# LimpBunion22/VIT-FPGA

Measured on AMD Instinct MI355X. Metric: images/sec ViT-B/16 224x224, batch 512 per GPU, higher is better.
Workload: dtype bf16; 1 GPU; vit_base 224x224x3 inference, 512 images per GPU resident in HBM, random-init weights (seed 0); global_batch=512, per_gpu_batch=512

## Files before the change

### vit-fpga_amd/csrc/kernels_attn.hip

```cpp
#include <type_traits>

#include "attn_common.h"

namespace vh {

template <typename T, typename TO = T>
__global__ void __launch_bounds__(1024, 4)
attention_kernel(const typename T::elem* __restrict__ qkv, typename TO::elem* __restrict__ out,
                 int tokens, int heads, int slabs, int ntiles) {
    using elem = typename T::elem;
    using vec8 = typename T::vec8;
    using vec4 = typename T::vec4;
    extern __shared__ __attribute__((aligned(16))) char smem[];
    const int kv_bytes = ntiles * 4096;

    const int lane = threadIdx.x & 63;
    const int wave = __builtin_amdgcn_readfirstlane(threadIdx.x >> 6);
    const int nw = blockDim.x >> 6;
    const int l31 = lane & 31, hl = lane >> 5;
    const int D = heads * 64;
    const int64_t ld = 3 * (int64_t)D;

    const int lr = lane >> 3, pc = lane & 7;
    const int ngroups = ntiles * 4;

    const int koff = l31 * 128;
    const int kswz = (l31 >> 1) & 7;
    const int g4 = lane >> 4, i16 = lane & 15, tq = i16 >> 2, tp = i16 & 3;
    const int vrow0 = 4 * (g4 >> 1) + tq;
    const int vcolb = (16 * (g4 & 1) + 4 * tp) * 2;

    const int item = blockIdx.x;
    const int bh = item / slabs, slab = item - bh * slabs;
    const int b = bh / heads, h = bh - b * heads;
    const int q0 = (slab * nw + wave) * 32;

    auto issue_kv = [&]() {
        const elem* base = qkv + (int64_t)b * tokens * ld + h * 64;
        for (int g = wave; g < ngroups; g += nw) {
            const int row = g * 8 + lr;
            const int rsrc = row < tokens ? row : tokens - 1;
            const elem* src = base + rsrc * ld;
            const int ck = pc ^ ((row >> 1) & 7);
            const int cv = pc ^ (((row >> 1) & 1) << 2);
            __builtin_amdgcn_global_load_lds((const void __attribute__((address_space(1)))*)(src + D + ck * 8),
                                             (void __attribute__((address_space(3)))*)(smem + g * 1024), 16, 0, 0);
            __builtin_amdgcn_global_load_lds((const void __attribute__((address_space(1)))*)(src + 2 * D + cv * 8),
                                             (void __attribute__((address_space(3)))*)(smem + kv_bytes + g * 1024), 16, 0, 0);
        }
    };
    vec8 qf[4];
    auto load_q = [&]() {
        int qrow = q0 + l31;
        qrow = qrow < tokens ? qrow : tokens - 1;
        const elem* qp = qkv + ((int64_t)b * tokens + qrow) * ld + h * 64 + 8 * hl;
#pragma unroll
        for (int ks = 0; ks < 4; ++ks) qf[ks] = *(const vec8*)(qp + 16 * ks);
    };
    issue_kv();
    load_q();

    asm volatile("s_waitcnt vmcnt(0)" ::: "memory");
    __syncthreads();
    const char* Ks = smem;
    const char* Vs = Ks + kv_bytes;

    if (q0 < tokens) {
        f32x16 o0, o1;
#pragma unroll
        for (int r = 0; r < 16; ++r) { o0[r] = 0.f; o1[r] = 0.f; }
        float m2 = -INFINITY;
        float lsum = 0.f;

        const char* kbase = Ks + koff;
        int kofs[4];
#pragma unroll
        for (int ks = 0; ks < 4; ++ks) kofs[ks] = ((2 * ks + hl) ^ kswz) << 4;
        const int vx = ((vrow0 >> 1) & 1) << 6;
        const char* vb0 = Vs + vrow0 * 128 + (vcolb ^ vx);
        const char* vb1 = Vs + vrow0 * 128 + ((vcolb + 64) ^ vx);

        auto qk = [&](int kt) {
            f32x16 s;
#pragma unroll
            for (int r = 0; r < 16; ++r) s[r] = 0.f;
            const char* kp = kbase + kt * 4096;
#pragma unroll
            for (int ks = 0; ks < 4; ++ks) s = T::mfma32(*(const vec8*)(kp + kofs[ks]), qf[ks], s);
            return s;
        };
        struct VFrag { vec8 f[2][2]; };
        auto load_v = [&](int kt) {
            VFrag v;
            const char* v0 = vb0 + kt * 4096;
            const char* v1 = vb1 + kt * 4096;
#pragma unroll
            for (int ks = 0; ks < 2; ++ks) {
                const vec4 a0 = T::tr_read(v0 + ks * 2048), c0 = T::tr_read(v0 + ks * 2048 + 1024);
                const vec4 a1 = T::tr_read(v1 + ks * 2048), c1 = T::tr_read(v1 + ks * 2048 + 1024);
#pragma unroll
                for (int j = 0; j < 4; ++j) { v.f[ks][0][j] = a0[j]; v.f[ks][0][4 + j] = c0[j]; v.f[ks][1][j] = a1[j]; v.f[ks][1][4 + j] = c1[j]; }
            }
            return v;
        };
        auto softmax_pv = [&](int kt, f32x16 s, const VFrag& vfr, auto masked) {
            if constexpr (decltype(masked)::value) {
#pragma unroll
                for (int r = 0; r < 16; ++r) {
                    const int key = kt * 32 + (r & 3) + 8 * (r >> 2) + 4 * hl;
                    if (key >= tokens) s[r] = -INFINITY;
                }
            }
            float mx = s[0];
#pragma unroll
            for (int r = 1; r < 16; ++r) mx = fmaxf(mx, s[r]);
            mx = cross_half_max(mx);
            const float mnew = fmaxf(m2, mx);
            if (__builtin_amdgcn_ballot_w64(mnew != m2)) {
                const float alpha = __builtin_amdgcn_exp2f(m2 - mnew);
                lsum *= alpha;
#pragma unroll
                for (int r = 0; r < 16; ++r) { o0[r] *= alpha; o1[r] *= alpha; }
                m2 = mnew;
            }
            float psum = 0.f;
#pragma unroll
            for (int r = 0; r < 16; ++r) {
                s[r] = __builtin_amdgcn_exp2f(s[r] - mnew);
                psum += s[r];
            }
            lsum += psum;
#pragma unroll
            for (int ks = 0; ks < 2; ++ks) {
                vec8 pf;
#pragma unroll
                for (int j = 0; j < 8; ++j) pf[j] = (elem)s[8 * ks + j];
                o0 = T::mfma32(vfr.f[ks][0], pf, o0);
                o1 = T::mfma32(vfr.f[ks][1], pf, o1);
            }
        };
        f32x16 s_cur = qk(0);
        for (int kt = 0; kt + 1 < ntiles; ++kt) {
            const VFrag vfr = load_v(kt);
            const f32x16 s_nxt = qk(kt + 1);
            softmax_pv(kt, s_cur, vfr, std::false_type{});
            s_cur = s_nxt;
        }
        {
            const VFrag vfr = load_v(ntiles - 1);
            softmax_pv(ntiles - 1, s_cur, vfr, std::true_type{});
        }

        const float ltot = cross_half_sum(lsum);
        const float inv = 1.0f / ltot;
        const int q = q0 + l31;
        if (q < tokens) {
            typename TO::elem* op = out + ((int64_t)b * tokens + q) * D + h * 64 + 4 * hl;
#pragma unroll
            for (int rg = 0; rg < 4; ++rg) {
                *(typename TO::vec4*)(op + 8 * rg) = pack4<TO>(o0[4 * rg] * inv, o0[4 * rg + 1] * inv, o0[4 * rg + 2] * inv, o0[4 * rg + 3] * inv);
                *(typename TO::vec4*)(op + 32 + 8 * rg) = pack4<TO>(o1[4 * rg] * inv, o1[4 * rg + 1] * inv, o1[4 * rg + 2] * inv, o1[4 * rg + 3] * inv);
            }
        }
    }
}

#ifndef VH_ATTN_ABL
#define VH_ATTN_ABL 0
#endif
__device__ __forceinline__ void ring_dma16(const void* base, uint32_t lane_off, uint32_t lds_addr) {
    asm_lds_dma16(base, lane_off, lds_addr);
}
#ifdef VH_DIAG_STAMPS
__device__ unsigned long long g_attn_diag[1024 * 16 * 16];
__device__ __forceinline__ unsigned long long attn_rt() {
    unsigned long long t;
    asm volatile("s_memrealtime %0\n\ts_waitcnt lgkmcnt(0)" : "=s"(t)::"memory");
    return t;
}
__device__ __forceinline__ unsigned long long attn_ct() {
    unsigned long long t;
    asm volatile("s_memtime %0\n\ts_waitcnt lgkmcnt(0)" : "=s"(t)::"memory");
    return t;
}
#define VH_ATT_T(i) do { __builtin_amdgcn_sched_barrier(0); const unsigned long long n_ = attn_ct(); ph_[i] += n_ - last_; last_ = n_; __builtin_amdgcn_sched_barrier(0); } while (0)
#else
#define VH_ATT_T(i) do { } while (0)
#endif
__device__ __forceinline__ void ring_wait_vm(int n) { wait_vm<40>(n); }
__device__ __forceinline__ void ring_wait_dma() {
    asm volatile("s_waitcnt vmcnt(0)" ::: "memory");
}

template <typename T, typename TO = T, bool QS = false, bool OTILE = false, bool IHM = false>
__global__ void __launch_bounds__(1024, 4)
attention_ring_kernel(const typename T::elem* __restrict__ qkv, typename TO::elem* __restrict__ out,
                      int tokens, int heads, int slabs, int ntiles, int nitems, unsigned int* __restrict__ ticket,
                      unsigned int heads_rcp, int64_t hm_rows) {
    using elem = typename T::elem;
    using vec8 = typename T::vec8;
    using vec4 = typename T::vec4;
    extern __shared__ __attribute__((aligned(16))) char smem[];
    const int G = (tokens + 7) >> 3, G2 = (G + 1) & ~1;
    const int kv_bytes = QS ? G * 1024 : ntiles * 4096;
    const int q_off = kv_bytes + (QS ? G2 * 1024 : kv_bytes);
    const uint32_t lds0 = (uint32_t)(uintptr_t)smem;

    const int lane = threadIdx.x & 63;
    const int wave = __builtin_amdgcn_readfirstlane(threadIdx.x >> 6);
    const int nw = blockDim.x >> 6;
    const int l31 = lane & 31, hl = lane >> 5;
    const int D = heads * 64;
    const int64_t ld = IHM ? 64 : 3 * (int64_t)D;
    const uint32_t koff2 = IHM ? (uint32_t)(hm_rows * D * 2) : (uint32_t)(D * 2);
    auto head_base = [&](int b, int h) {
        if constexpr (IHM) return qkv + ((int64_t)h * hm_rows + (int64_t)b * tokens) * 64;
        else return qkv + (int64_t)b * tokens * ld + h * 64;
    };

    auto kv_base = [&](int item) {
        if (QS) {
            const int b = (heads == 1 ? item : (int)__umulhi((unsigned)item, heads_rcp)), h = item - b * heads;
            return head_base(b, h);
        }
        const int bh = item / slabs;
        const int b = bh / heads, h = bh - b * heads;
        return head_base(b, h);
    };
    auto issue_tile = [&](const elem* base, int t) {
        int ln = lane;
        asm volatile("" : "+v"(ln));
        const int lr_ = ln >> 3, pc_ = ln & 7;
        const int g = 4 * t + wave;
        const int gk = QS && g >= G ? G - 1 : g, gv = QS && g >= G2 ? G2 - 1 : g;
        const int rowk = gk * 8 + lr_, rowv = gv * 8 + lr_;
        const int rk = rowk < tokens ? rowk : tokens - 1;
        const int rv = rowv < tokens ? rowv : tokens - 1;
        const int ck = pc_ ^ ((rowk >> 1) & 7);
        const int cv = pc_ ^ (((rowv >> 1) & 1) << 2);
        const uint32_t ok = (uint32_t)(rk * (int)ld + ck * 8) * 2u + koff2;
        const uint32_t ov = (uint32_t)(rv * (int)ld + cv * 8) * 2u + 2u * koff2;
        ring_dma16(base, ok, lds0 + gk * 1024);
        ring_dma16(base, ov, lds0 + kv_bytes + gv * 1024);
    };
    auto issue_q = [&](const elem* base) {
        int ln = lane;
        asm volatile("" : "+v"(ln));
        const int lr_ = ln >> 3, pc_ = ln & 7;
        for (int j = 0; j < nw; ++j) {
            const int g = 4 * j + wave;
            const int row = g * 8 + lr_;
            const int rsrc = row < tokens ? row : tokens - 1;
            const int ck = pc_ ^ ((row >> 1) & 7);
            ring_dma16(base, (uint32_t)(rsrc * (int)ld + ck * 8) * 2u, lds0 + q_off + g * 1024);
        }
    };
    auto load_q = [&](int item, vec8 (&qf)[4]) {
        const int bh = item / slabs, slab = item - bh * slabs;
        const int b = bh / heads, h = bh - b * heads;
        int qrow = (slab * nw + wave) * 32 + l31;
        qrow = qrow < tokens ? qrow : tokens - 1;
        const elem* qp = head_base(b, h) + (int64_t)qrow * ld + 8 * hl;
        asm volatile("global_load_dwordx4 %0, %4, off\n\tglobal_load_dwordx4 %1, %4, off offset:32\n\t"
                     "global_load_dwordx4 %2, %4, off offset:64\n\tglobal_load_dwordx4 %3, %4, off offset:96"
                     : "=&v"(qf[0]), "=&v"(qf[1]), "=&v"(qf[2]), "=&v"(qf[3]) : "v"(qp) : "memory");
    };

    const int kswz = (l31 >> 1) & 7;
    const int g4 = lane >> 4, i16 = lane & 15, tq = i16 >> 2, tp = i16 & 3;
    const int vrow0 = 4 * (g4 >> 1) + tq;
    const int vcolb = (16 * (g4 & 1) + 4 * tp) * 2;
    const int k0 = l31 * 128 + ((hl ^ kswz) << 4);
    const int vx = ((vrow0 >> 1) & 1) << 6;
    const int v0 = kv_bytes + vrow0 * 128 + (vcolb ^ vx);

    const int stride = (int)gridDim.x;
    int item = blockIdx.x * slabs;
    const elem* cbase = kv_base(item);
    vec8 qf[4];
    if (wave < 4) {
        if (QS) issue_q(cbase);
        for (int t = 0; t < ntiles; ++t) issue_tile(cbase, t);
    }
    if (!QS) load_q(item, qf);
    bool first = true;
    constexpr int NST = 4;
    const int w_top = 2 * (ntiles - 2) + NST, w_t1 = 2 * (ntiles - 3) + NST + 2, w_mid = 2 * ntiles + nw - 4 + NST, w_last = nw + 2 + 2 * (ntiles - 3);
    bool stored = false;

#ifdef VH_DIAG_STAMPS
    const unsigned long long rt0_ = attn_rt();
    unsigned int dbg_[3] = {0xffffffffu, 0xffffffffu, 0xffffffffu};
    int dbg_n_ = 0;
    unsigned long long ph_[10] = {0, 0, 0, 0, 0, 0, 0, 0, 0, 0}, last_ = attn_ct();
#endif
    const bool dyn = QS && ticket != nullptr && nw >= 5;
    const int tk_off = q_off + 4 * nw * 1024;
    unsigned int tkv = 0;
    while (true) {
        const int slab_now = QS ? 0 : item - (item / slabs) * slabs;
        const bool last_slab = QS || slab_now + 1 == slabs;
        int next = QS ? item + stride : (last_slab ? (item / slabs + stride) * slabs : item + 1);
        if (QS && dyn && !first) {
            if (wave == nw - 1) {
                if (stored) asm volatile("s_waitcnt vmcnt(%0)" :: "n"(NST) : "memory");
                else asm volatile("s_waitcnt vmcnt(0)" ::: "memory");
                asm volatile("" : "+v"(tkv));
                if (lane == 0) *(volatile unsigned int __attribute__((address_space(3)))*)(uintptr_t)(lds0 + tk_off) = 2u * (unsigned)stride + tkv;
            }
        }
        const int b = QS ? (heads == 1 ? item : (int)__umulhi((unsigned)item, heads_rcp)) : (item / slabs) / heads;
        const int slab = slab_now;
        const int h = (QS ? item : item / slabs) - b * heads;
        const int q0 = (slab * nw + wave) * 32;

        VH_ATT_T(7);
        if (QS) {
            ring_wait_vm(first ? 0 : w_top);
        } else {
            if (first || !stored) asm volatile("s_waitcnt vmcnt(0)" ::: "memory");
            else asm volatile("s_waitcnt vmcnt(%0)" :: "n"(NST) : "memory");
            asm volatile("" : "+v"(qf[0]), "+v"(qf[1]), "+v"(qf[2]), "+v"(qf[3]));
        }
        VH_ATT_T(0);
        ring_barrier();
        VH_ATT_T(1);
        if (QS && dyn && !first) next = __builtin_amdgcn_readfirstlane(*(volatile const int __attribute__((address_space(3)))*)(uintptr_t)(lds0 + tk_off));
#if defined(VH_DIAG_STAMPS) && defined(VH_ATTN_TKDBG)
        if (QS && dyn && !first) { if (dbg_n_ < 3) dbg_[dbg_n_++] = (unsigned)next; next = item + stride; }
#endif
        const bool has_next = (unsigned)next < (unsigned)nitems;
        const bool refill = has_next && last_slab;
        const elem* nbase = kv_base(has_next ? next : item);
        if (QS && dyn && has_next && wave == nw - 1 && lane == 0) {
            asm_atomic_add_ret_issue(ticket, 1u, tkv);
        }
        if (!(VH_ATTN_ABL & 2) && !first && slab == 0 && wave < 4) issue_tile(cbase, ntiles - 1);
        if (QS) {
            int qa = q_off + wave * 4096 + k0;
            if constexpr (!std::is_same<T, TO>::value) {
                int ln = lane;
                asm volatile("" : "+v"(ln));
                const int r31 = ln & 31;
                qa = q_off + wave * 4096 + r31 * 128 + ((((ln >> 5)) ^ ((r31 >> 1) & 7)) << 4);
            }
#pragma unroll
            for (int ks = 0; ks < 4; ++ks) qf[ks] = *(const vec8*)(smem + (qa ^ (ks << 5)));
        }

        f32x16 o0, o1;
#pragma unroll
        for (int r = 0; r < 16; ++r) { o0[r] = 0.f; o1[r] = 0.f; }
        float negm = 0.f;
        float lsum = 0.f;

        auto qk = [&](int kt, float init) {
            int ka = k0 + kt * 4096;
            if constexpr (!std::is_same<T, TO>::value) asm volatile("" : "+v"(ka));
            vec8 kf[4];
#pragma unroll
            for (int ks = 0; ks < 4; ++ks) {
                if (VH_ATTN_ABL & 32) kf[ks] = qf[ks]; else if (VH_ATTN_ABL & 128) kf[ks] = *(const vec8*)(smem + ((ka ^ (ks << 5)) & 0x3ff0)); else
                kf[ks] = *(const vec8*)(smem + (ka ^ (ks << 5)));
            }
            __builtin_amdgcn_sched_barrier(0);
            typedef float f32x2 __attribute__((ext_vector_type(2)));
            typedef float f32x8 __attribute__((ext_vector_type(8)));
            const f32x2 i2 = {init, init};
            f32x2 p[8];
#pragma unroll
            for (int i = 0; i < 8; ++i) asm volatile("v_mov_b64 %0, %1" : "=v"(p[i]) : "v"(i2));
            const f32x4 q0 = __builtin_shufflevector(p[0], p[1], 0, 1, 2, 3), q1 = __builtin_shufflevector(p[2], p[3], 0, 1, 2, 3);
            const f32x4 q2 = __builtin_shufflevector(p[4], p[5], 0, 1, 2, 3), q3 = __builtin_shufflevector(p[6], p[7], 0, 1, 2, 3);
            const f32x8 h0 = __builtin_shufflevector(q0, q1, 0, 1, 2, 3, 4, 5, 6, 7), h1 = __builtin_shufflevector(q2, q3, 0, 1, 2, 3, 4, 5, 6, 7);
            f32x16 s = __builtin_shufflevector(h0, h1, 0, 1, 2, 3, 4, 5, 6, 7, 8, 9, 10, 11, 12, 13, 14, 15);
#pragma unroll
            for (int ks = 0; ks < 4; ++ks) {
                if (VH_ATTN_ABL & 16) s[ks] += (float)kf[ks][0] * (float)qf[ks][0];
                else s = T::mfma32(kf[ks], qf[ks], s);
            }
            return s;
        };
        struct VFrag { vec8 f[2][2]; };
        auto load_v = [&](int kt) {
            VFrag v;
            if (VH_ATTN_ABL & 32) { for (int ks = 0; ks < 2; ++ks) { v.f[ks][0] = qf[ks]; v.f[ks][1] = qf[ks + 2]; } return v; }
            const char* p0 = smem + (v0 + kt * 4096);
            const char* p1 = smem + ((v0 + kt * 4096) ^ 64);
#pragma unroll
            for (int ks = 0; ks < 2; ++ks) {
                const vec4 a0 = T::tr_read(p0 + ks * 2048), c0 = T::tr_read(p0 + ks * 2048 + 1024);
                const vec4 a1 = T::tr_read(p1 + ks * 2048), c1 = T::tr_read(p1 + ks * 2048 + 1024);
#pragma unroll
                for (int j = 0; j < 4; ++j) { v.f[ks][0][j] = a0[j]; v.f[ks][0][4 + j] = c0[j]; v.f[ks][1][j] = a1[j]; v.f[ks][1][4 + j] = c1[j]; }
            }
            return v;
        };
        auto softmax_pv = [&](int kt, f32x16& s, const VFrag& vfr, auto first_c, auto tail_c) {
            constexpr bool FIRST = decltype(first_c)::value, TAIL = decltype(tail_c)::value;
            int ng = 4;
            if constexpr (TAIL) {
                const int valid = tokens - kt * 32;
                ng = (valid + 7) >> 3;
#pragma unroll
                for (int g = 0; g < 4; ++g)
                    if (g < ng) {
#pragma unroll
                        for (int j = 0; j < 4; ++j)
                            if (8 * g + j + 4 * hl >= valid) s[4 * g + j] = -INFINITY;
                    }
            }
            float mx = -INFINITY;
#pragma unroll
            for (int g = 0; g < 4; ++g)
                if (!TAIL || g < ng) {
#pragma unroll
                    for (int j = 0; j < 4; ++j) mx = fmaxf(mx, s[4 * g + j]);
                }
            if (VH_ATTN_ABL & 64) mx = s[kt & 15];
            else
            mx = cross_half_max(mx);
            if constexpr (FIRST) {
                negm = -mx;
#pragma unroll
                for (int r = 0; r < 16; ++r) s[r] -= mx;
            } else if (__builtin_amdgcn_ballot_w64(mx > kTau)) {
                const float delta = fmaxf(mx, 0.f);
                const float alpha = __builtin_amdgcn_exp2f(-delta);
                negm -= delta;
                lsum *= alpha;
#pragma unroll
                for (int r = 0; r < 16; ++r) { o0[r] *= alpha; o1[r] *= alpha; s[r] -= delta; }
            }
            typedef float f32x2 __attribute__((ext_vector_type(2)));
            f32x2 psum = {0.f, 0.f};
#pragma unroll
            for (int g = 0; g < 4; ++g) {
                if (!TAIL || g < ng) {
#pragma unroll
                    for (int j = 0; j < 4; ++j) s[4 * g + j] = (VH_ATTN_ABL & 1) ? s[4 * g + j] * 0.001f + 1.0f : __builtin_amdgcn_exp2f(s[4 * g + j]);
                    psum += f32x2{s[4 * g], s[4 * g + 1]};
                    psum += f32x2{s[4 * g + 2], s[4 * g + 3]};
                } else {
#pragma unroll
                    for (int j = 0; j < 4; ++j) s[4 * g + j] = 0.f;
                }
            }
            lsum += psum[0] + psum[1];
#pragma unroll
            for (int ks = 0; ks < 2; ++ks) {
                if (!TAIL || 2 * ks < ng) {
                    vec8 pf;
#pragma unroll
                    for (int j = 0; j < 8; ++j) pf[j] = (elem)s[8 * ks + j];
                    if (VH_ATTN_ABL & 8) { o0[ks] += (float)pf[0]; o1[ks] += (float)vfr.f[ks][0][0] + (float)vfr.f[ks][1][0]; }
                    else {
                    o0 = T::mfma32(vfr.f[ks][0], pf, o0);
                    o1 = T::mfma32(vfr.f[ks][1], pf, o1);
                    }
                }
            }
        };

        {
            const VFrag vfr = load_v(0);
            f32x16 sc = qk(0, 0.f);
            softmax_pv(0, sc, vfr, std::true_type{}, std::false_type{});
        }
        VH_ATT_T(2);
        for (int kt = 1; kt + 1 < ntiles; ++kt) {
            if (QS) ring_wait_vm(kt == 1 ? w_t1 : !has_next ? 0 : w_mid);
            VH_ATT_T(4);
            if (!(VH_ATTN_ABL & 4)) ring_barrier();
            VH_ATT_T(3);
            if (QS && kt == 1 && has_next && wave < 4) issue_q(nbase);
            if (!(VH_ATTN_ABL & 2) && refill && wave < 4) issue_tile(nbase, kt - 1);
            const VFrag vfr = load_v(kt);
            f32x16 sc = qk(kt, negm);
            softmax_pv(kt, sc, vfr, std::false_type{}, std::false_type{});
        }
        VH_ATT_T(4);
        if (QS) ring_wait_vm(!has_next ? 0 : w_last);
        else ring_wait_dma();
        VH_ATT_T(5);
        if (!(VH_ATTN_ABL & 4)) ring_barrier();
        VH_ATT_T(6);
        if (!(VH_ATTN_ABL & 2) && refill && wave < 4) issue_tile(nbase, ntiles - 2);
        {
            const VFrag vfr = load_v(ntiles - 1);
            f32x16 sc = qk(ntiles - 1, negm);
            if (!QS && has_next) load_q(next, qf);
            softmax_pv(ntiles - 1, sc, vfr, std::false_type{}, std::true_type{});
            VH_ATT_T(8);

            const float ltot = cross_half_sum(lsum);
            const float inv = __builtin_amdgcn_rcpf(ltot);
            const int q = q0 + l31;
            if constexpr (sizeof(typename TO::elem) == 2) {
                const int64_t mrow = (int64_t)b * tokens + (q < tokens ? q : tokens - 1);
                typename TO::elem* const op = OTILE ? out + ((mrow >> 4) * (D >> 3) + h * 8 + hl) * 128 + (mrow & 15) * 8
                                                    : out + mrow * D + h * 64 + 8 * hl;
                constexpr int CH = OTILE ? 128 : 8;
#pragma unroll
                for (int db = 0; db < 2; ++db) {
                    const f32x16& o = db ? o1 : o0;
#pragma unroll
                    for (int rg = 0; rg < 4; rg += 2) {
                        const u32x2 ga = __builtin_bit_cast(u32x2, pack4<TO>(o[4 * rg] * inv, o[4 * rg + 1] * inv, o[4 * rg + 2] * inv, o[4 * rg + 3] * inv));
                        const u32x2 gb = __builtin_bit_cast(u32x2, pack4<TO>(o[4 * rg + 4] * inv, o[4 * rg + 5] * inv, o[4 * rg + 6] * inv, o[4 * rg + 7] * inv));
                        const auto sx = __builtin_amdgcn_permlane32_swap(ga[0], gb[0], false, false);
                        const auto sy = __builtin_amdgcn_permlane32_swap(ga[1], gb[1], false, false);
                        if (q < tokens) *(u32x4*)(op + (4 * db + rg) * CH) = u32x4{sx[0], sy[0], sx[1], sy[1]};
                    }
                }
            } else {
                const int64_t mrow = (int64_t)b * tokens + (q < tokens ? q : tokens - 1);
                typename TO::elem* const op = OTILE ? out + ((mrow >> 4) * (D >> 4) + h * 4) * 256 + (mrow & 15) * 16 + 8 * hl
                                                    : out + mrow * D + h * 64 + 8 * hl;
#pragma unroll
                for (int db = 0; db < 2; ++db) {
                    const f32x16& o = db ? o1 : o0;
#pragma unroll
                    for (int rg = 0; rg < 4; rg += 2) {
                        const uint32_t ga = pack4<TO>(o[4 * rg] * inv, o[4 * rg + 1] * inv, o[4 * rg + 2] * inv, o[4 * rg + 3] * inv);
                        const uint32_t gb = pack4<TO>(o[4 * rg + 4] * inv, o[4 * rg + 5] * inv, o[4 * rg + 6] * inv, o[4 * rg + 7] * inv);
                        const auto sx = __builtin_amdgcn_permlane32_swap(ga, gb, false, false);
                        if (q < tokens) *(u32x2*)(op + (OTILE ? (2 * db + (rg >> 1)) * 256 : 32 * db + 8 * rg)) = u32x2{sx[0], sx[1]};
                    }
                }
            }
        }
        VH_ATT_T(9);
        if (!has_next) break;
        stored = q0 < tokens;
        item = next;
        cbase = nbase;
        first = false;
    }
#ifdef VH_DIAG_STAMPS
    VH_ATT_T(7);
    if (lane == 0 && blockIdx.x < 1024) {
#pragma unroll
        for (int i = 0; i < 10; ++i) g_attn_diag[((size_t)blockIdx.x * 16 + wave) * 16 + i] = ph_[i];
        unsigned int hw;
        asm volatile("s_getreg_b32 %0, hwreg(HW_REG_HW_ID)" : "=s"(hw));
        unsigned int xcc;
        asm volatile("s_getreg_b32 %0, hwreg(HW_REG_XCC_ID)" : "=s"(xcc));
        g_attn_diag[((size_t)blockIdx.x * 16 + wave) * 16 + 10] = rt0_;
        g_attn_diag[((size_t)blockIdx.x * 16 + wave) * 16 + 11] = attn_rt();
        g_attn_diag[((size_t)blockIdx.x * 16 + wave) * 16 + 12] = ((unsigned long long)xcc << 32) | hw;
        for (int i = 0; i < 3; ++i) g_attn_diag[((size_t)blockIdx.x * 16 + wave) * 16 + 13 + i] = dbg_[i];
    }
#endif
}

#ifdef VH_DIAG_STAMPS
extern "C" int vh_diag_attn_read(unsigned long long* host, int n_words) {
    return (int)hipMemcpyFromSymbol(host, HIP_SYMBOL(g_attn_diag), (size_t)n_words * 8);
}
#endif

size_t attention_lds_bytes(int tokens) { return (size_t)((tokens + 31) / 32) * 8192; }

enum class AttnForm { NONE, ONE_SHOT, RING, RING_QS };
struct AttnPlan { AttnForm form; int slabs, nw; size_t lds; };
static AttnPlan attn_plan(int tokens, bool out_tiled, bool in_head_major) {
    constexpr int kMaxWaves = 16;
    const int ntiles = (tokens + 31) / 32;
    const int slabs = (ntiles + kMaxWaves - 1) / kMaxWaves, nw = (ntiles + slabs - 1) / slabs;
    const size_t one = attention_lds_bytes(tokens);
    if (one > 160 * 1024) return {AttnForm::NONE, slabs, nw, 0};
    const int G = (tokens + 7) / 8, G2 = (G + 1) & ~1;
    const size_t qs_lds = (size_t)(G + G2 + 4 * nw) * 1024 + 16;
    if (slabs == 1 && nw >= 4 && 2 * qs_lds <= 160 * 1024) return {AttnForm::RING_QS, slabs, nw, qs_lds};
    if (ntiles >= 3 && nw >= 4) return {AttnForm::RING, slabs, nw, one};
    if (out_tiled || in_head_major) return {AttnForm::NONE, slabs, nw, 0};
    return {AttnForm::ONE_SHOT, slabs, nw, one};
}
bool attention_tiled_applies(int batch, int tokens, int heads) {
    (void)batch;
    return attn_plan(tokens, true, false).form != AttnForm::NONE && heads % 2 == 0;
}

template <typename T, typename TO = T, bool OTILE = false, bool IHM = false>
static hipError_t launch_attn_t(const void* qkv, int batch, int tokens, int heads, void* out, unsigned int* ticket, hipStream_t s, bool tk_zeroed,
                                int64_t hm_rows = 0) {
    const AttnPlan p = attn_plan(tokens, OTILE, IHM);
    if (p.form == AttnForm::NONE) return hipErrorInvalidValue;
    const int ntiles = (tokens + 31) / 32, slabs = p.slabs, nw = p.nw;
    const int nitems = batch * heads * slabs;
    const int num_cu = device_num_cu();
    if (!num_cu) return hipErrorUnknown;
    if (p.form == AttnForm::RING_QS) {
        auto k = attention_ring_kernel<T, TO, true, OTILE, IHM>;
        static LdsDone lds_done;
        if (hipError_t e = ensure_dynamic_lds((const void*)k, p.lds, lds_done); e != hipSuccess) return e;
        const int grid = nitems < 2 * num_cu ? nitems : 2 * num_cu;
        unsigned int* tk = nw >= 5 && nitems > 2 * grid ? ticket : nullptr;
        if (tk && !tk_zeroed) { if (hipError_t e = hipMemsetAsync(tk, 0, sizeof(unsigned int), s); e != hipSuccess) return e; }
        const unsigned int heads_rcp = (unsigned int)(((1ull << 32) + (unsigned)heads - 1) / (unsigned)heads);
        hipLaunchKernelGGL(k, dim3(grid), dim3(nw * 64), p.lds, s, (const typename T::elem*)qkv, (typename TO::elem*)out,
                           tokens, heads, slabs, ntiles, nitems, tk, heads_rcp, hm_rows);
        return hipGetLastError();
    }
    if (p.form == AttnForm::RING) {
        auto k = attention_ring_kernel<T, TO, false, OTILE, IHM>;
        static LdsDone lds_done;
        if (hipError_t e = ensure_dynamic_lds((const void*)k, p.lds, lds_done); e != hipSuccess) return e;
        const int per_cu = (int)(160 * 1024 / p.lds);
        int grid = num_cu * (per_cu < 1 ? 1 : (per_cu > 2 ? 2 : per_cu));
        if (grid > batch * heads) grid = batch * heads;
        hipLaunchKernelGGL(k, dim3(grid), dim3(nw * 64), p.lds, s, (const typename T::elem*)qkv, (typename TO::elem*)out,
                           tokens, heads, slabs, ntiles, nitems, (unsigned int*)nullptr, 0u, hm_rows);
        return hipGetLastError();
    }
    if constexpr (OTILE || IHM) return hipErrorInvalidValue;
    else {
        auto k = attention_kernel<T, TO>;
        static LdsDone lds_done;
        if (hipError_t e = ensure_dynamic_lds((const void*)k, p.lds, lds_done); e != hipSuccess) return e;
        hipLaunchKernelGGL(k, dim3(nitems), dim3(nw * 64), p.lds, s, (const typename T::elem*)qkv, (typename TO::elem*)out,
                           tokens, heads, slabs, ntiles);
        return hipGetLastError();
    }
}

template <typename T>
__global__ void __launch_bounds__(256)
attention_cls_kernel(const typename T::elem* __restrict__ qkv, typename T::elem* __restrict__ out, int batch, int tokens, int heads) {
    using elem = typename T::elem;
    using vec8 = typename T::vec8;
    constexpr int MAXT = 1024;
    __shared__ float sc[4][MAXT];
    const int lane = threadIdx.x & 63, wv = threadIdx.x >> 6;
    const int item = blockIdx.x * 4 + wv;
    if (item >= batch * heads) return;
    const int b = item / heads, h = item - b * heads;
    const int D = heads * 64;
    const int64_t ld = 3 * (int64_t)D;
    const elem* const base = qkv + (int64_t)b * tokens * ld + h * 64;
    const int g = lane >> 3, c = lane & 7;
    float q[8];
    {
        const vec8 v = *(const vec8*)(base + c * 8);
#pragma unroll
        for (int j = 0; j < 8; ++j) q[j] = (float)v[j];
    }
    float mx = -INFINITY;
    constexpr int U = 4;
    for (int t0 = 0; t0 < tokens; t0 += 8 * U) {
        vec8 v[U];
#pragma unroll
        for (int u = 0; u < U; ++u) {
            const int t = t0 + 8 * u + g;
            v[u] = *(const vec8*)(base + (t < tokens ? t : tokens - 1) * ld + D + c * 8);
        }
#pragma unroll
        for (int u = 0; u < U; ++u) {
            const int t = t0 + 8 * u + g;
            float sv = 0.f;
#pragma unroll
            for (int j = 0; j < 8; ++j) sv = fmaf(q[j], (float)v[u][j], sv);
            sv += __shfl_xor(sv, 1); sv += __shfl_xor(sv, 2); sv += __shfl_xor(sv, 4);
            if (t < tokens) {
                if (c == 0) sc[wv][t] = sv;
                mx = fmaxf(mx, sv);
            }
        }
    }
#pragma unroll
    for (int o = 32; o > 0; o >>= 1) mx = fmaxf(mx, __shfl_xor(mx, o));
    __builtin_amdgcn_s_waitcnt(0xC07F);
    float sum = 0.f;
    for (int t = lane; t < tokens; t += 64) {
        const float p = __builtin_amdgcn_exp2f(sc[wv][t] - mx);
        sc[wv][t] = p;
        sum += p;
    }
#pragma unroll
    for (int o = 32; o > 0; o >>= 1) sum += __shfl_xor(sum, o);
    __builtin_amdgcn_s_waitcnt(0xC07F);
    float acc[8] = {0.f, 0.f, 0.f, 0.f, 0.f, 0.f, 0.f, 0.f};
    for (int t0 = 0; t0 < tokens; t0 += 8 * U) {
        vec8 v[U];
#pragma unroll
        for (int u = 0; u < U; ++u) {
            const int t = t0 + 8 * u + g;
            v[u] = *(const vec8*)(base + (t < tokens ? t : tokens - 1) * ld + 2 * D + c * 8);
        }
#pragma unroll
        for (int u = 0; u < U; ++u) {
            const int t = t0 + 8 * u + g;
            const float p = t < tokens ? sc[wv][t] : 0.f;
#pragma unroll
            for (int j = 0; j < 8; ++j) acc[j] = fmaf(p, (float)v[u][j], acc[j]);
        }
    }
#pragma unroll
    for (int j = 0; j < 8; ++j) {
        acc[j] += __shfl_xor(acc[j], 8); acc[j] += __shfl_xor(acc[j], 16); acc[j] += __shfl_xor(acc[j], 32);
    }
    if (g == 0) {
        const float r = 1.0f / sum;
        vec8 o;
#pragma unroll
        for (int j = 0; j < 8; ++j) o[j] = (elem)(acc[j] * r);
        *(vec8*)(out + (int64_t)b * D + h * 64 + c * 8) = o;
    }
}
hipError_t launch_attention_cls(const void* qkv16, int batch, int tokens, int heads, void* out16, int dtype, hipStream_t s) {
    if (batch <= 0 || tokens <= 0 || tokens > 1024 || heads <= 0) return hipErrorInvalidValue;
    const dim3 grid((unsigned)((batch * heads + 3) / 4));
    if (dtype == VH_DTYPE_BF16)
        hipLaunchKernelGGL(attention_cls_kernel<BF16>, grid, dim3(256), 0, s, (const BF16::elem*)qkv16, (BF16::elem*)out16, batch, tokens, heads);
    else if (dtype == VH_DTYPE_FP16)
        hipLaunchKernelGGL(attention_cls_kernel<FP16>, grid, dim3(256), 0, s, (const FP16::elem*)qkv16, (FP16::elem*)out16, batch, tokens, heads);
    else
        return hipErrorInvalidValue;
    return hipGetLastError();
}

hipError_t launch_attention(const void* qkv16, int batch, int tokens, int heads, void* out16, int dtype,
                            unsigned int* ticket, hipStream_t s, bool ticket_zeroed, bool out_tiled, int64_t in_hm_rows) {
    if (batch <= 0 || tokens <= 0 || heads <= 0) return hipErrorInvalidValue;
    if (in_hm_rows) {
        if (!out_tiled || in_hm_rows < (int64_t)batch * tokens || in_hm_rows * heads * 64 * 4 >= (1ll << 32)) return hipErrorInvalidValue;
        if (!attention_tiled_applies(batch, tokens, heads)) return hipErrorInvalidValue;
        if (dtype == VH_DTYPE_FP8) return launch_attn_t<BF16, E4M3, true, true>(qkv16, batch, tokens, heads, out16, ticket, s, ticket_zeroed, in_hm_rows);
        return dtype == VH_DTYPE_BF16 ? launch_attn_t<BF16, BF16, true, true>(qkv16, batch, tokens, heads, out16, ticket, s, ticket_zeroed, in_hm_rows)
                                      : launch_attn_t<FP16, FP16, true, true>(qkv16, batch, tokens, heads, out16, ticket, s, ticket_zeroed, in_hm_rows);
    }
    if (out_tiled) {
        if (!attention_tiled_applies(batch, tokens, heads)) return hipErrorInvalidValue;
        if (dtype == VH_DTYPE_FP8) return launch_attn_t<BF16, E4M3, true>(qkv16, batch, tokens, heads, out16, ticket, s, ticket_zeroed);
        return dtype == VH_DTYPE_BF16 ? launch_attn_t<BF16, BF16, true>(qkv16, batch, tokens, heads, out16, ticket, s, ticket_zeroed)
                                      : launch_attn_t<FP16, FP16, true>(qkv16, batch, tokens, heads, out16, ticket, s, ticket_zeroed);
    }
    if (attention_lds_bytes(tokens) > 160 * 1024) return launch_attention_hd(qkv16, batch, tokens, heads, 64, out16, dtype, s);
    if (dtype == VH_DTYPE_FP8) return launch_attn_t<BF16, E4M3>(qkv16, batch, tokens, heads, out16, ticket, s, ticket_zeroed);
    return dtype == VH_DTYPE_BF16 ? launch_attn_t<BF16>(qkv16, batch, tokens, heads, out16, ticket, s, ticket_zeroed)
                                  : launch_attn_t<FP16>(qkv16, batch, tokens, heads, out16, ticket, s, ticket_zeroed);
}

}
```

Before: 28770 images/s.

## Merge near-empty last KV tile into the second-to-last tile pass in attention

Adds an MT variant of the staged-Q ring attention kernel. It is used when the final 32-token KV tile holds at most 8 valid tokens, which is the case for ViT's 197 tokens. The last two tiles are handled in one merged pass: both QK products are issued together, the tail tile's score is computed inside the rescale step, and one barrier/wait stage is dropped. The refill is brought forward one tile, and the vmcnt wait thresholds are adjusted to match. The aim is to cut per-item synchronisation and latency spent on the nearly empty tail tile, at the cost of more register pressure and more complex wait-count bookkeeping.

Result: no change. 28860 images/s, median of 6 (+0.3%).

```diff
diff --git a/vit-fpga_amd/csrc/kernels_attn.hip b/vit-fpga_amd/csrc/kernels_attn.hip
--- a/vit-fpga_amd/csrc/kernels_attn.hip
+++ b/vit-fpga_amd/csrc/kernels_attn.hip
@@ -192,7 +192,7 @@
     asm volatile("s_waitcnt vmcnt(0)" ::: "memory");
 }
 
-template <typename T, typename TO = T, bool QS = false, bool OTILE = false, bool IHM = false>
+template <typename T, typename TO = T, bool QS = false, bool OTILE = false, bool IHM = false, bool MT = false>
 __global__ void __launch_bounds__(1024, 4)
 attention_ring_kernel(const typename T::elem* __restrict__ qkv, typename TO::elem* __restrict__ out,
                       int tokens, int heads, int slabs, int ntiles, int nitems, unsigned int* __restrict__ ticket,
@@ -200,6 +200,7 @@
     using elem = typename T::elem;
     using vec8 = typename T::vec8;
     using vec4 = typename T::vec4;
+    static_assert(!MT || QS, "the merged tail pass exists in the staged-Q form only");
     extern __shared__ __attribute__((aligned(16))) char smem[];
     const int G = (tokens + 7) >> 3, G2 = (G + 1) & ~1;
     const int kv_bytes = QS ? G * 1024 : ntiles * 4096;
@@ -285,7 +286,8 @@
     if (!QS) load_q(item, qf);
     bool first = true;
     constexpr int NST = 4;
-    const int w_top = 2 * (ntiles - 2) + NST, w_t1 = 2 * (ntiles - 3) + NST + 2, w_mid = 2 * ntiles + nw - 4 + NST, w_last = nw + 2 + 2 * (ntiles - 3);
+    const int w_top = 2 * (ntiles - 2 - MT) + NST, w_t1 = 2 * (ntiles - 3 - MT) + NST + 2 + 2 * MT, w_mid = 2 * ntiles + nw - 4 + NST,
+              w_last = nw + 2 + 2 * (ntiles - 3 - MT);
     bool stored = false;
 
 #ifdef VH_DIAG_STAMPS
@@ -335,9 +337,12 @@
         if (QS && dyn && has_next && wave == nw - 1 && lane == 0) {
             asm_atomic_add_ret_issue(ticket, 1u, tkv);
         }
+        if (MT && !(VH_ATTN_ABL & 2) && !first && wave < 4) issue_tile(cbase, ntiles - 2);
         if (!(VH_ATTN_ABL & 2) && !first && slab == 0 && wave < 4) issue_tile(cbase, ntiles - 1);
         if (QS) {
-            int qa = q_off + wave * 4096 + k0;
+            int qk0 = k0;
+            if constexpr (MT) asm volatile("" : "+v"(qk0));
+            int qa = q_off + wave * 4096 + qk0;
             if constexpr (!std::is_same<T, TO>::value) {
                 int ln = lane;
                 asm volatile("" : "+v"(ln));
@@ -354,16 +359,22 @@
         float negm = 0.f;
         float lsum = 0.f;
 
-        auto qk = [&](int kt, float init) {
-            int ka = k0 + kt * 4096;
+        struct KFrag { vec8 f[4]; };
+        auto k_read = [&](int kt) {
+            int kk = k0;
+            if constexpr (MT) asm volatile("" : "+v"(kk));
+            int ka = kk + kt * 4096;
             if constexpr (!std::is_same<T, TO>::value) asm volatile("" : "+v"(ka));
-            vec8 kf[4];
+            KFrag k;
 #pragma unroll
             for (int ks = 0; ks < 4; ++ks) {
-                if (VH_ATTN_ABL & 32) kf[ks] = qf[ks]; else if (VH_ATTN_ABL & 128) kf[ks] = *(const vec8*)(smem + ((ka ^ (ks << 5)) & 0x3ff0)); else
-                kf[ks] = *(const vec8*)(smem + (ka ^ (ks << 5)));
-            }
-            __builtin_amdgcn_sched_barrier(0);
+                if (VH_ATTN_ABL & 32) k.f[ks] = qf[ks]; else if (VH_ATTN_ABL & 128) k.f[ks] = *(const vec8*)(smem + ((ka ^ (ks << 5)) & 0x3ff0)); else
+                k.f[ks] = *(const vec8*)(smem + (ka ^ (ks << 5)));
+            }
+            return k;
+        };
+        auto k_mul = [&](const KFrag& k, float init) {
+            const vec8 (&kf)[4] = k.f;
             typedef float f32x2 __attribute__((ext_vector_type(2)));
             typedef float f32x8 __attribute__((ext_vector_type(8)));
             const f32x2 i2 = {init, init};
@@ -381,12 +392,20 @@
             }
             return s;
         };
+        auto qk = [&](int kt, float init) {
+            const KFrag k = k_read(kt);
+            __builtin_amdgcn_sched_barrier(0);
+            return k_mul(k, init);
+        };
         struct VFrag { vec8 f[2][2]; };
         auto load_v = [&](int kt) {
             VFrag v;
             if (VH_ATTN_ABL & 32) { for (int ks = 0; ks < 2; ++ks) { v.f[ks][0] = qf[ks]; v.f[ks][1] = qf[ks + 2]; } return v; }
-            const char* p0 = smem + (v0 + kt * 4096);
-            const char* p1 = smem + ((v0 + kt * 4096) ^ 64);
+            int va = v0;
+            if constexpr (MT) asm volatile("" : "+v"(va));
+            va += kt * 4096;
+            const char* p0 = smem + va;
+            const char* p1 = smem + (va ^ 64);
 #pragma unroll
             for (int ks = 0; ks < 2; ++ks) {
                 const vec4 a0 = T::tr_read(p0 + ks * 2048), c0 = T::tr_read(p0 + ks * 2048 + 1024);
@@ -396,12 +415,14 @@
             }
             return v;
         };
+        [[maybe_unused]] f32x16 st;
         auto softmax_pv = [&](int kt, f32x16& s, const VFrag& vfr, auto first_c, auto tail_c) {
-            constexpr bool FIRST = decltype(first_c)::value, TAIL = decltype(tail_c)::value;
+            constexpr int MODE = (int)decltype(tail_c)::value;
+            constexpr bool FIRST = decltype(first_c)::value, TAIL = MODE == 1 || MODE == 3;
             int ng = 4;
             if constexpr (TAIL) {
                 const int valid = tokens - kt * 32;
-                ng = (valid + 7) >> 3;
+                ng = MODE == 3 ? 1 : (valid + 7) >> 3;
 #pragma unroll
                 for (int g = 0; g < 4; ++g)
                     if (g < ng) {
@@ -431,6 +452,7 @@
                 lsum *= alpha;
 #pragma unroll
                 for (int r = 0; r < 16; ++r) { o0[r] *= alpha; o1[r] *= alpha; s[r] -= delta; }
+                if constexpr (MODE == 2) st = k_mul(k_read(kt + 1), negm);
             }
             typedef float f32x2 __attribute__((ext_vector_type(2)));
             f32x2 psum = {0.f, 0.f};
@@ -468,7 +490,7 @@
             softmax_pv(0, sc, vfr, std::true_type{}, std::false_type{});
         }
         VH_ATT_T(2);
-        for (int kt = 1; kt + 1 < ntiles; ++kt) {
+        for (int kt = 1; kt + 1 + MT < ntiles; ++kt) {
             if (QS) ring_wait_vm(kt == 1 ? w_t1 : !has_next ? 0 : w_mid);
             VH_ATT_T(4);
             if (!(VH_ATTN_ABL & 4)) ring_barrier();
@@ -479,19 +501,36 @@
             f32x16 sc = qk(kt, negm);
             softmax_pv(kt, sc, vfr, std::false_type{}, std::false_type{});
         }
-        VH_ATT_T(4);
-        if (QS) ring_wait_vm(!has_next ? 0 : w_last);
-        else ring_wait_dma();
-        VH_ATT_T(5);
-        if (!(VH_ATTN_ABL & 4)) ring_barrier();
-        VH_ATT_T(6);
-        if (!(VH_ATTN_ABL & 2) && refill && wave < 4) issue_tile(nbase, ntiles - 2);
-        {
+        if constexpr (MT) {
+            ring_wait_vm(!has_next ? 0 : w_last);
+            VH_ATT_T(4);
+            if (!(VH_ATTN_ABL & 4)) ring_barrier();
+            VH_ATT_T(3);
+            if (!(VH_ATTN_ABL & 2) && refill && wave < 4) issue_tile(nbase, ntiles - 3);
+            f32x16 sc = qk(ntiles - 2, negm);
+            st = qk(ntiles - 1, negm);
+            __builtin_amdgcn_sched_barrier(0);
+            const VFrag vfr = load_v(ntiles - 2);
+            softmax_pv(ntiles - 2, sc, vfr, std::false_type{}, std::integral_constant<int, 2>{});
+            const VFrag vft = load_v(ntiles - 1);
+            asm volatile("" : "+v"(st));
+            softmax_pv(ntiles - 1, st, vft, std::false_type{}, std::integral_constant<int, 3>{});
+            VH_ATT_T(4);
+        } else {
+            VH_ATT_T(4);
+            if (QS) ring_wait_vm(!has_next ? 0 : w_last);
+            else ring_wait_dma();
+            VH_ATT_T(5);
+            if (!(VH_ATTN_ABL & 4)) ring_barrier();
+            VH_ATT_T(6);
+            if (!(VH_ATTN_ABL & 2) && refill && wave < 4) issue_tile(nbase, ntiles - 2);
             const VFrag vfr = load_v(ntiles - 1);
             f32x16 sc = qk(ntiles - 1, negm);
             if (!QS && has_next) load_q(next, qf);
             softmax_pv(ntiles - 1, sc, vfr, std::false_type{}, std::true_type{});
             VH_ATT_T(8);
+        }
+        {
 
             const float ltot = cross_half_sum(lsum);
             const float inv = __builtin_amdgcn_rcpf(ltot);
@@ -592,8 +631,12 @@
     const int num_cu = device_num_cu();
     if (!num_cu) return hipErrorUnknown;
     if (p.form == AttnForm::RING_QS) {
-        auto k = attention_ring_kernel<T, TO, true, OTILE, IHM>;
-        static LdsDone lds_done;
+        const int valid = tokens - 32 * (ntiles - 1);
+        constexpr bool kHasMerged = std::is_same<T, TO>::value;
+        const bool merged_tail = kHasMerged && valid <= 8 && ntiles >= 4;
+        auto k = merged_tail ? attention_ring_kernel<T, TO, true, OTILE, IHM, kHasMerged> : attention_ring_kernel<T, TO, true, OTILE, IHM, false>;
+        static LdsDone lds_done_form[2];
+        LdsDone& lds_done = lds_done_form[merged_tail];
         if (hipError_t e = ensure_dynamic_lds((const void*)k, p.lds, lds_done); e != hipSuccess) return e;
         const int grid = nitems < 2 * num_cu ? nitems : 2 * num_cu;
         unsigned int* tk = nw >= 5 && nitems > 2 * grid ? ticket : nullptr;
```
